# Julia-Tempering/Pigeons.jl

Measured on AMD Instinct MI355X. Metric: replica-steps/sec (explore+swap), toy_mvn d=1024, n_chains=1024; round-trip rate, higher is better.
Workload: dtype f64

## Files before the change

### pigeons.jl_amd/csrc/pte_slice8.hpp

```cpp
#pragma once
#include "pte_slice7.hpp"

namespace pte {

#ifndef PTE_S8_BD
#define PTE_S8_BD 3
#endif
#ifndef PTE_S8_BS
#define PTE_S8_BS 9
#endif
constexpr int S8_BD = PTE_S8_BD;

#ifndef PTE_S8_WAVES
#define PTE_S8_WAVES 4
#endif
template <int NLU, int S8_BS, int WINDOW, int DBL_MODE>
__device__ __forceinline__ void slice8_body(EngineDev e, SliceParams sp, const int64_t cl) {
    using namespace s7;
    constexpr int WIN = WINDOW, REFILL_AT = WINDOW - PTE_S7_MARGIN;
    constexpr bool FAST = (DBL_MODE == 2);
    static_assert(CAP_ITERS >= S8_BS, "lane 0 must be able to run past the speculative budget");
#ifndef PTE_S8_BLK
#define PTE_S8_BLK 256
#endif
    constexpr int BLK = PTE_S8_BLK, CPB = BLK / 64;
    constexpr bool HOLD_POLICY = (WIN == 512);
    __shared__ struct {
        double u[WIN];
        double e[WIN];
        double x[BLK];
        double we[256];
        unsigned long long ke[256];
        unsigned policy[HOLD_POLICY ? 2 : 0];
    } sm;
    double (&s_u)[WIN] = sm.u; double (&s_e)[WIN] = sm.e; double (&s_x)[BLK] = sm.x; double (&s_we)[256] = sm.we; unsigned long long (&s_ke)[256] = sm.ke;
    const int lane = lane_id();
#ifdef PTE_PROFILE_WAVES
    const uint64_t wave_t0 = __builtin_amdgcn_s_memrealtime();
#endif
    for (int i = lane; i < 256; i += 64) { s_we[i] = ZIG_WE[i]; s_ke[i] = ZIG_KE[i]; }
    if constexpr (HOLD_POLICY) sm.policy[0] = g_rng_policy;
    const auto exp_seq = [&](SeqRng &rs) __attribute__((always_inline)) -> double {
        if constexpr (HOLD_POLICY)
            return randexp_from_raw_hot(rs, rs.next(), [&]() __attribute__((always_inline)) -> unsigned {
                return (unsigned)__builtin_amdgcn_readfirstlane((int)*(const volatile __attribute__((address_space(3))) unsigned *)&sm.policy[0]); });
        else
            return randexp_seq(rs);
    };
    __syncthreads();
    if (cl >= e.K) return;
    const int64_t c = e.c0 + cl;
    const int slot = e.slot_of_chain[cl];
    if (is_ref_chain(e, c)) {
        iid_refresh_recorded<NLU>(e, cl, c, slot, e.sd[c], lane);
        return;
    }
    const double lp_before = lp_before_explore(e, c, slot);
    const int64_t d = e.d;
    double *xrow = e.x + (int64_t)slot * e.ld;
    const int B = (int)((d + 63) >> 6);
    const double nhp = e.nhp[c];
    const double inv_nhp = 1.0 / nhp;
    const double inv_abs_nhp = -inv_nhp * (1.0 + 1e-6);
    const double w = sp.w;
    const double w11 = 1.1 * sp.w;
    const int cap_iters = min(sp.max_iter, CAP_ITERS);
    const int kcap = min(sp.p, 20);
    const bool shr_more = S8_BS < cap_iters;
    constexpr bool HAND_SHRINK = (S8_BS == PTE_S8_BS && S8_BS >= 6 && S8_BS <= 10);
    constexpr bool N_IS_KN = (DBL_MODE == 2) && HAND_SHRINK;

    const int hg = s7_level(lane);
    const int hrel = s7_pick(LO, hg, 0) + lane - s7_pick(BASE, hg, 0);

    const int succ_lo = s7_pick(LO, hg + 1, 0), succ_wd = s7_pick(WD, hg + 1, 0), succ_base = s7_pick(BASE, hg + 1, 0);
    const int succ_off = hrel - succ_lo;
    const int word_c = 0x10000 - succ_off;
    const int word_c9 = (1 << 20) - succ_off * 512;
    const uint64_t seed_in = e.rng[2 * slot];

    double BS = 0.0;
    for (int b = 0; b < B; ++b) {
        int64_t i = 64 * (int64_t)b + lane;
        double v = (i < d) ? xrow[i] : 0.0;
        double s = wave_sum_dpp(v * v);
        if (lane == b) BS = s;
    }
    double S = upper_tree_root<NLU>(BS);
    if (nhp * S == -INFINITY) { if (lane == 0) set_error(e, ERR_SLICE_SUPPORT, (int)c, -1); return; }

    uint64_t wseed = e.rng[2 * slot];
    const uint64_t gamma = e.rng[2 * slot + 1];
    int p = 0;
    uint64_t gamma_inv = gamma;
    for (int k = 0; k < 5; ++k) gamma_inv *= 2ull - gamma * gamma_inv;
    double wsum = 0.0;
    typedef unsigned mask2_t __attribute__((ext_vector_type(2)));
    typedef unsigned slow_mask_t __attribute__((ext_vector_type(WIN / 32)));
    typedef double draws8_t __attribute__((ext_vector_type(8)));
    typedef double draws2_t __attribute__((ext_vector_type(2)));
    slow_mask_t slow_w;
    auto fill_window = [&]() __attribute__((always_inline)) {
        __syncthreads();
        double acc = 0.0;
#pragma unroll
        for (int k = 0; k < WIN / 64; ++k) {
            const int i = 64 * k + lane;
            const uint64_t r = mix64(wseed + (uint64_t)(i + 1) * gamma);
            const uint64_t ri = r & MASK52;
            const int idx = (int)(ri & 0xFF);
            const bool fast = ri < s_ke[idx];
            const double ev = (double)ri * s_we[idx];
            s_u[i] = u52_to_unit(r);
            s_e[i] = fast ? ev : __longlong_as_double(0x7ff8000000000000LL);
            acc += fast ? ev : 0.0;
            const uint64_t sb = ballot64(!fast);
            slow_w[2 * k] = (unsigned)sb; slow_w[2 * k + 1] = (unsigned)(sb >> 32);
        }
        wsum = wave_sum_dpp(acc);
        p = 0;
        __syncthreads();
    };
    fill_window();

    int dbl_z0 = 0, dbl_z1 = 0, dbl_one_hi = 0x3ff00000;
    if constexpr (DBL_MODE == 2) asm volatile("" : "+v"(dbl_z0), "+v"(dbl_z1), "+v"(dbl_one_hi));

    long long steps_sum = 0, fb_draws = 0, ex_total = 0;
    int steps_n = 0, acc_sum = 0, acc_n = 0, n_fb = 0;
    int err = 0, err_coord = -1;
#ifdef PTE_PROFILE_SECTIONS
    long long prof[20] = {0, 0, 0, 0, 0, 0, 0, 0, 0, 0, 0, 0, 0, 0, 0, 0, 0, 0, 0, 0};
#endif

    for (int pass = 0; pass < sp.n_passes && !err; ++pass) {
        for (int b = 0; BLK * (int64_t)b < d && !err; ++b) {
            const int64_t base = BLK * (int64_t)b;
            const int nl = (int)min((int64_t)BLK, d - base);
#pragma unroll
            for (int k = 0; k < CPB; ++k) s_x[64 * k + lane] = (64 * k + lane < nl) ? xrow[base + 64 * k + lane] : 0.0;
            __builtin_amdgcn_wave_barrier();
            double Sest = S * (1.0 + 1e-6) + wsum * inv_abs_nhp;
            int l = 0, l_end = nl;
            do {
                PROF_T(t0);
                if (__builtin_expect(p > REFILL_AT, 0)) { PROF_T(tr0); wseed += (uint64_t)p * gamma; fill_window(); Sest = Sest * (1.0 + 1e-6) + wsum * inv_abs_nhp; PROF_T(tr1); PROF_ADD(16, tr1 - tr0); PROF_ADD(17, 1); }
                const bool active = (l + hg) < nl;
                const double xold = s_x[(l + hg) & (BLK - 1)];
                int idx0 = p + hrel;
                double E = s_e[idx0];
                double u0 = s_u[idx0 + 1];
                double Vd[S8_BD];
#pragma unroll
                for (int it = 0; it < S8_BD; ++it) Vd[it] = s_u[idx0 + 2 + it];
                int ua = 0;
                if constexpr (DBL_MODE == 2) ua = (int)(uintptr_t)(const __attribute__((address_space(3))) double *)&s_u[idx0];
                int ex0 = 0;
                int cnt_base = 2;
                asm volatile("" : "+v"(cnt_base));
                if constexpr (DBL_MODE == 2) asm volatile("" : "+s"(ex0));
                unsigned slow_b;
                if constexpr (WIN == 512)
                    asm("s_lshr_b32 m0, %[p], 5\n" "s_nop 0\n" "s_movrels_b32 %[o], s84\n" "s_lshr_b32 %[o], %[o], %[p]"
                        : [o] "=&s"(slow_b) : [p] "s"(p), "{s[84:99]}"(slow_w) : "m0", "scc");
                else
                    asm("s_lshr_b32 m0, %[p], 5\n" "s_nop 0\n" "s_movrels_b32 %[o], s84\n" "s_lshr_b32 %[o], %[o], %[p]"
                        : [o] "=&s"(slow_b) : [p] "s"(p), "{s[84:91]}"(slow_w) : "m0", "scc");
                static_assert(WIN == 512 || WIN == 256, "the slow-path mask is sixteen or eight dwords");
                if (__builtin_expect((slow_b & 1u) != 0u, 0)) {
                    PROF_T(ts0);
                    SeqRng rs{wseed + (uint64_t)p * gamma, gamma};
                    const double Ex = exp_seq(rs);
                    const int used = (int)((rs.seed - (wseed + (uint64_t)p * gamma)) * gamma_inv);
                    if (used <= 17) {
                        ex0 = used - 1;
                        if (lane == 0) { E = Ex; idx0 += ex0; cnt_base = 2 + ex0; ua += 8 * ex0; }
                        Sest += Ex * inv_abs_nhp;
                        ex_total += ex0;
                        u0 = s_u[idx0 + 1];
#pragma unroll
                        for (int it = 0; it < S8_BD; ++it) Vd[it] = s_u[idx0 + 2 + it];
                    }
#ifdef PTE_PROFILE_SECTIONS
                    asm volatile("" :: "v"(E), "v"(u0), "v"(Vd[S8_BD - 1]), "v"(Sest));
#endif
                    PROF_T(ts1); PROF_ADD(18, ts1 - ts0); PROF_ADD(19, 1);
                }
                const double Enh = E * inv_nhp;
                const double Q = __builtin_fma(xold, xold, -Enh);
                const double Bq = Sest + fabs(Q);
                double dmin = fabs(Enh);
                auto test = [&](double v) __attribute__((always_inline)) -> double {
                    const double d = __builtin_fma(v, v, -Q);
                    dmin = fmin(dmin, fabs(d));
                    return d;
                };
                double LL = xold - w * u0;
                double RR = LL + w;
                double dL = test(LL), dR = test(RR);
                int kd = 0;
                double dmin_lr = 0.0;
                unsigned need_l0 = 0u;
                uint64_t need_m = 0ull;
                double thr2 = 0.0, mthr = 0.0, W = 0.0;
                int n = 0;
                uint64_t act_m = 0ull;
                draws8_t ud8 = 0.0; draws2_t ud2 = 0.0;
#if PTE_S8_BD >= 1 && PTE_S8_BD <= 4 && !defined(PTE_S8_DOUBLING_SELECTS)
                if constexpr (DBL_MODE == 2) {
                    double t_, wd_;
                    int sLh_, sRh_;
                    uint64_t sv_, sx_;
                    mask2_t sd_;
#define PTE_S8_CSTEP(V) \
                    "v_cmp_ge_f64 vcc, 0.5, " V "\n" \
                    "v_min_f64 v[102:103], v[114:115], v[116:117]\n" \
                    "v_cmpx_gt_f64_e64 %[sx], 0, v[102:103]\n" \
                    "v_add_f64 v[112:113], v[98:99], -v[96:97]\n" \
                    "v_add_u32 %[kd], 1, %[kd]\n" \
                    "v_add_u32 %[ua], 8, %[ua]\n" \
                    "v_cndmask_b32 v119, 0, %[one], vcc\n" \
                    "v_cndmask_b32 v121, %[one], v118, vcc\n" \
                    "v_fma_f64 v[96:97], -v[118:119], v[112:113], v[96:97]\n" \
                    "v_fma_f64 v[98:99], v[120:121], v[112:113], v[98:99]\n" \
                    "v_fma_f64 v[114:115], v[96:97], v[96:97], -v[110:111]\n" \
                    "v_fma_f64 v[116:117], v[98:99], v[98:99], -v[110:111]\n"
#define PTE_S8_CFOLD \
                    "v_min_f64 v[104:105], v[104:105], |v[114:115]|\n" \
                    "v_min_f64 v[104:105], v[104:105], |v[116:117]|\n"
#if PTE_S8_BS == 6
#define PTE_S8_UREADS_TAIL
#elif PTE_S8_BS == 7
#define PTE_S8_UREADS_TAIL "ds_read_b64 v[136:137], %[ua] offset:64\n"
#elif PTE_S8_BS == 8
#define PTE_S8_UREADS_TAIL "ds_read2_b64 v[136:139], %[ua] offset0:8 offset1:9\n"
#elif PTE_S8_BS == 9
#define PTE_S8_UREADS_TAIL "ds_read2_b64 v[136:139], %[ua] offset0:8 offset1:9\n" "ds_read_b64 v[140:141], %[ua] offset:80\n"
#else
#define PTE_S8_UREADS_TAIL "ds_read2_b64 v[136:139], %[ua] offset0:8 offset1:9\n" "ds_read2_b64 v[140:143], %[ua] offset0:10 offset1:11\n"
#endif
                    asm volatile("s_mov_b64 %[sv], exec\n"
#if PTE_S8_BD >= 2
                                 PTE_S8_CSTEP("%[V0]") PTE_S8_CFOLD
#endif
#if PTE_S8_BD >= 3
                                 PTE_S8_CSTEP("%[V1]") PTE_S8_CFOLD
#endif
#if PTE_S8_BD >= 4
                                 PTE_S8_CSTEP("%[V2]") PTE_S8_CFOLD
#endif
                                 PTE_S8_CSTEP("%[VL]")
                                 "s_mov_b64 exec, %[sv]\n"
                                 "ds_read2_b64 v[124:127], %[ua] offset0:2 offset1:3\n"
                                 "ds_read2_b64 v[128:131], %[ua] offset0:4 offset1:5\n"
                                 "ds_read2_b64 v[132:135], %[ua] offset0:6 offset1:7\n"
                                 PTE_S8_UREADS_TAIL
                                 "v_min_f64 v[102:103], v[114:115], v[116:117]\n"
                                 "v_cmp_gt_f64_e64 %[sd], 0, v[102:103]\n"
                                 PTE_S8_CFOLD
                                 "v_add_f64 %[mthr], %[Sest], |v[110:111]|\n"
                                 "v_max_f64 %[thr], |v[96:97]|, |v[98:99]|\n"
                                 "v_cmp_gt_i32_e64 %[act], %[nl], %[lg]\n"
                                 "v_add3_u32 v106, %[cb], %[so], %[kd]\n"
                                 "v_mul_f64 %[mthr], %[mthr], %[c_m]\n"
                                 "v_mul_f64 %[thr], %[thr], %[c_t]\n"
                                 "v_add_f64 v[112:113], v[98:99], -v[96:97]\n"
                                 : "+{v[96:97]}"(LL), "+{v[98:99]}"(RR), "+{v[114:115]}"(dL), "+{v[116:117]}"(dR), "+{v[104:105]}"(dmin), [kd] "+v"(kd), [ua] "+v"(ua),
                                   "=&{v[102:103]}"(t_), "=&{v[112:113]}"(wd_), "=&{v119}"(sLh_), "=&{v121}"(sRh_), [sv] "=&s"(sv_), [sx] "=&s"(sx_), [sd] "=&s"(sd_),
                                   "=&{v[124:139]}"(ud8), "=&{v[140:143]}"(ud2), [mthr] "=&v"(mthr), [thr] "=&v"(thr2), "=&{v106}"(n), [act] "=&s"(act_m)
                                 : "{v[110:111]}"(Q), "{v118}"(dbl_z0), "{v120}"(dbl_z1), [one] "v"(dbl_one_hi),
                                   [V0] "v"(Vd[0]), [V1] "v"(Vd[S8_BD > 2 ? 1 : 0]), [V2] "v"(Vd[S8_BD > 3 ? 2 : 0]), [VL] "v"(Vd[S8_BD - 1]),
                                   [Sest] "v"(Sest), [nl] "s"(nl), [lg] "v"(l + hg), [cb] "v"(cnt_base), [so] "v"(succ_off), [c_m] "s"(2e-12), [c_t] "s"(1e-6)
                                 : "vcc", "scc");
#undef PTE_S8_CSTEP
#undef PTE_S8_CFOLD
#undef PTE_S8_UREADS_TAIL
                    dmin_lr = t_; W = wd_;
                    need_m = (uint64_t)sd_.x | ((uint64_t)sd_.y << 32); need_l0 = __builtin_amdgcn_readfirstlane(sd_.x);
                } else
                if (DBL_MODE == 1 && sp.p >= S8_BD) {
                    double t_, wd_;
                    uint64_t sv_, sv2_;
#define PTE_S8_DSTEP(V) \
                    "v_min_f64 %[t], %[dL], %[dR]\n" \
                    "v_cmp_gt_f64 vcc, 0, %[t]\n" \
                    "s_and_saveexec_b64 %[sv], vcc\n" \
                    "v_add_u32 %[kd], 1, %[kd]\n" \
                    "v_add_f64 %[wd], %[RR], -%[LL]\n" \
                    "v_cmp_ge_f64 vcc, 0.5, " V "\n" \
                    "s_and_saveexec_b64 %[sv2], vcc\n" \
                    "v_add_f64 %[LL], %[LL], -%[wd]\n" \
                    "v_fma_f64 %[dL], %[LL], %[LL], -%[Q]\n" \
                    "v_min_f64 %[dmin], %[dmin], |%[dL]|\n" \
                    "s_andn2_b64 exec, %[sv2], exec\n" \
                    "v_add_f64 %[RR], %[RR], %[wd]\n" \
                    "v_fma_f64 %[dR], %[RR], %[RR], -%[Q]\n" \
                    "v_min_f64 %[dmin], %[dmin], |%[dR]|\n" \
                    "s_mov_b64 exec, %[sv]\n"
                    asm volatile(PTE_S8_DSTEP("%[V0]")
#if PTE_S8_BD >= 2
                                 PTE_S8_DSTEP("%[V1]")
#endif
#if PTE_S8_BD >= 3
                                 PTE_S8_DSTEP("%[V2]")
#endif
#if PTE_S8_BD >= 4
                                 PTE_S8_DSTEP("%[V3]")
#endif
                                 : [LL] "+v"(LL), [RR] "+v"(RR), [dL] "+v"(dL), [dR] "+v"(dR), [dmin] "+v"(dmin), [kd] "+v"(kd),
                                   [t] "=&v"(t_), [wd] "=&v"(wd_), [sv] "=&s"(sv_), [sv2] "=&s"(sv2_)
                                 : [Q] "v"(Q), [V0] "v"(Vd[0]), [V1] "v"(Vd[S8_BD > 1 ? 1 : 0]), [V2] "v"(Vd[S8_BD > 2 ? 2 : 0]), [V3] "v"(Vd[S8_BD > 3 ? 3 : 0])
                                 : "vcc", "scc");
#undef PTE_S8_DSTEP
                } else
#endif
#pragma unroll
                for (int it = 0; it < S8_BD; ++it) {
                    const bool need = (fmin(dL, dR) < 0.0) && it < sp.p;
                    const double V = Vd[it];
                    kd += need ? 1 : 0;
                    const bool left = V <= 0.5;
                    const double wd = RR - LL;
                    if constexpr (DBL_MODE == 0) {
                        const double sL = (need && left) ? 1.0 : 0.0, sR = (need && !left) ? 1.0 : 0.0;
                        LL = __builtin_fma(-sL, wd, LL);
                        RR = __builtin_fma(sR, wd, RR);
                        dL = __builtin_fma(LL, LL, -Q);
                        dR = __builtin_fma(RR, RR, -Q);
                        dmin = fmin(dmin, fmin(fabs(dL), fabs(dR)));
                    } else {
                        const double cand = left ? (LL - wd) : (RR + wd);
                        const double dc = __builtin_fma(cand, cand, -Q);
                        dmin = need ? fmin(dmin, fabs(dc)) : dmin;
                        const bool nl_ = need && left, nr_ = need && !left;
                        LL = nl_ ? cand : LL;
                        RR = nr_ ? cand : RR;
                        dL = nl_ ? dc : dL;
                        dR = nr_ ? dc : dR;
                    }
                }
#if !(PTE_S8_BD >= 1 && PTE_S8_BD <= 4) || defined(PTE_S8_DOUBLING_SELECTS)
                static_assert(DBL_MODE != 2, "PTE_S8_DBL_MODE == 2 needs the v_cmpx doubling block: 1 <= PTE_S8_BD <= 4 and no PTE_S8_DOUBLING_SELECTS");
#endif
                if constexpr (DBL_MODE != 2) dmin_lr = fmin(dL, dR);
                unsigned more_dbl;
                if constexpr (FAST) more_dbl = need_l0 & 1u;
                else more_dbl = ballot64(lane == 0 && (dmin_lr < 0.0) && kd < kcap) != 0ull ? 1u : 0u;
                if (__builtin_expect(more_dbl != 0u, 0)) {
                    bool need = (lane == 0);
                    while (need) {
                        const double V = s_u[idx0 + 2 + kd];
                        kd += 1;
                        const bool left = V <= 0.5;
                        const double wd = RR - LL;
                        const double cand = left ? (LL - wd) : (RR + wd);
                        const double dc = test(cand);
                        LL = left ? cand : LL;
                        RR = left ? RR : cand;
                        dL = left ? dc : dL;
                        dR = left ? dR : dc;
                        need = (kd < kcap) && (fmin(dL, dR) < 0.0);
                    }
                    asm volatile("" : "+v"(dL), "+v"(dR), "+v"(kd));
                    dmin_lr = fmin(dL, dR);
                    if constexpr (FAST) {
                        dmin_lr = (kd >= sp.p) ? 0.0 : dmin_lr;
                        need_m = ballot64(dmin_lr < 0.0);
                        need_l0 = (unsigned)need_m;
                        thr2 = 1e-6 * fmax(fabs(LL), fabs(RR));
                        n = cnt_base + kd + succ_off;
                        W = RR - LL;
                        const double *un = &s_u[idx0 + 2 + kd];
#pragma unroll
                        for (int k = 0; k < 8; ++k) ud8[k] = (k < S8_BS) ? un[k] : 0.0;
#pragma unroll
                        for (int k = 8; k < 10; ++k) ud2[k - 8] = (k < S8_BS) ? un[k] : 0.0;
                        asm volatile("" : "+{v[124:139]}"(ud8), "+{v[140:143]}"(ud2));
                    }
                }
                const bool dbl_ok = FAST ? !__builtin_amdgcn_inverse_ballot_w64(need_m) : !((kd < sp.p) && (dmin_lr < 0.0));
                if constexpr (DBL_MODE != 2) thr2 = 1e-6 * fmax(fabs(LL), fabs(RR));
#ifdef PTE_PROFILE_SECTIONS
                asm volatile("" :: "v"(LL), "v"(RR), "v"(kd), "v"(thr2));
#endif
                PROF_T(t1); PROF_ADD(0, t1 - t0);
                static_assert(DBL_MODE != 2 || HAND_SHRINK, "PTE_S8_DBL_MODE == 2 hands its draws to the hand-written shrinkage block: 6 <= PTE_S8_BS <= 10");
                const double *us = &s_u[idx0 + 2 + kd];
                double u[S8_BS];
                if constexpr (DBL_MODE != 2) {
#pragma unroll
                    for (int k = 0; k < S8_BS; ++k) u[k] = us[k];
                }
                if constexpr (DBL_MODE != 2) mthr = 2e-12 * Bq;
                int kn0 = cnt_base + kd + succ_off;
                uint64_t pre_ok;
                if constexpr (FAST) pre_ok = 0ull;
                else pre_ok = ballot64(active && dbl_ok);
                double Lbar = LL, Rbar = RR, xf = xold;
                if constexpr (!N_IS_KN) n = 0;
                bool fin = false;
                unsigned unf_l0 = 0u;
                uint64_t unf_m = 0ull;
                if constexpr (S8_BS == PTE_S8_BS && S8_BS >= 6 && S8_BS <= 10) {
                    double t_;
                    mask2_t unf_mask;
                    uint64_t exec_save;
#define PTE_S8_STEP_W \
                    "v_add_f64 v[112:113], v[98:99], -v[96:97]\n"
#define PTE_S8_STEP(U) PTE_S8_STEP_W PTE_S8_STEP_U(U)
#define PTE_S8_STEP_U(U) \
                    "v_mul_f64 v[102:103], " U ", v[112:113]\n" \
                    "v_add_f64 v[100:101], v[96:97], v[102:103]\n" \
                    "v_cmp_lt_f64 vcc, v[100:101], v[108:109]\n" \
                    "v_fma_f64 v[102:103], v[100:101], v[100:101], -v[110:111]\n" \
                    "v_add_u32 v106, 1, v106\n" \
                    "v_cndmask_b32 v96, v96, v100, vcc\n" \
                    "v_cndmask_b32 v97, v97, v101, vcc\n" \
                    "v_cndmask_b32 v98, v100, v98, vcc\n" \
                    "v_cndmask_b32 v99, v101, v99, vcc\n" \
                    "v_min_f64 v[104:105], v[104:105], |v[102:103]|\n" \
                    "v_cmpx_ngt_f64 vcc, 0, v[102:103]\n"
                    if constexpr (DBL_MODE == 2) {
#if defined(PTE_S8_ONE_WAIT) || defined(PTE_PROFILE_SECTIONS)
#define PTE_S8_WAIT(K) "s_waitcnt lgkmcnt(0)\n"
#else
#define PTE_S8_WAIT(K) "s_waitcnt lgkmcnt(" #K ")\n"
#endif
#if PTE_S8_BS >= 9
#define PTE_S8_W1 4
#define PTE_S8_W3 3
#define PTE_S8_W5 2
#define PTE_S8_W7 1
#elif PTE_S8_BS >= 7
#define PTE_S8_W1 3
#define PTE_S8_W3 2
#define PTE_S8_W5 1
#define PTE_S8_W7 0
#else
#define PTE_S8_W1 2
#define PTE_S8_W3 1
#define PTE_S8_W5 0
#endif
#define PTE_S8_WAIT_(K) PTE_S8_WAIT(K)
                    asm volatile(".p2align 3\n"
                                 "s_mov_b64 %[sv], exec\n"
                                 "s_andn2_b64 %[pre], %[act], %[need]\n"
                                 PTE_S8_WAIT_(PTE_S8_W1) PTE_S8_STEP_U("v[124:125]") PTE_S8_STEP("v[126:127]")
                                 PTE_S8_STEP_W PTE_S8_WAIT_(PTE_S8_W3) PTE_S8_STEP_U("v[128:129]") PTE_S8_STEP("v[130:131]")
                                 PTE_S8_STEP_W PTE_S8_WAIT_(PTE_S8_W5) PTE_S8_STEP_U("v[132:133]") PTE_S8_STEP("v[134:135]")
#if PTE_S8_BS >= 7
                                 PTE_S8_STEP_W PTE_S8_WAIT_(PTE_S8_W7) PTE_S8_STEP_U("v[136:137]")
#endif
#if PTE_S8_BS >= 8
                                 PTE_S8_STEP("v[138:139]")
#endif
#if PTE_S8_BS >= 9
                                 PTE_S8_STEP_W PTE_S8_WAIT_(0) PTE_S8_STEP_U("v[140:141]")
#endif
#if PTE_S8_BS >= 10
                                 PTE_S8_STEP("v[142:143]")
#endif
                                 "s_mov_b64 %[unf], exec\n"
                                 "s_mov_b64 exec, %[sv]\n"
                                 "s_nop 3\n"
                                 : "+{v[96:97]}"(Lbar), "+{v[98:99]}"(Rbar), "=&{v[100:101]}"(xf), "=&{v[102:103]}"(t_),
                                   "+{v[104:105]}"(dmin), "+{v106}"(n), "+{v[112:113]}"(W), [unf] "=&s"(unf_mask), [sv] "=&s"(exec_save), [pre] "=&s"(pre_ok)
                                 : "{v[108:109]}"(xold), "{v[110:111]}"(Q), "{v[124:139]}"(ud8), "{v[140:143]}"(ud2), [act] "s"(act_m), [need] "s"(need_m)
                                 : "vcc", "scc");
#undef PTE_S8_WAIT
#undef PTE_S8_WAIT_
#undef PTE_S8_W1
#undef PTE_S8_W3
#undef PTE_S8_W5
#undef PTE_S8_W7
                    } else
                    asm volatile(".p2align 3\n"
                                 "s_mov_b64 %[sv], exec\n"
                                 PTE_S8_STEP("%[u0]") PTE_S8_STEP("%[u1]") PTE_S8_STEP("%[u2]") PTE_S8_STEP("%[u3]")
                                 PTE_S8_STEP("%[u4]") PTE_S8_STEP("%[u5]")
#if PTE_S8_BS >= 7
                                 PTE_S8_STEP("%[u6]")
#endif
#if PTE_S8_BS >= 8
                                 PTE_S8_STEP("%[u7]")
#endif
#if PTE_S8_BS >= 9
                                 PTE_S8_STEP("%[u8]")
#endif
#if PTE_S8_BS >= 10
                                 PTE_S8_STEP("%[u9]")
#endif
                                 "s_mov_b64 %[unf], exec\n"
                                 "s_mov_b64 exec, %[sv]\n"
                                 "s_nop 3\n"
                                 : "+{v[96:97]}"(Lbar), "+{v[98:99]}"(Rbar), "=&{v[100:101]}"(xf), "=&{v[102:103]}"(t_),
                                   "+{v[104:105]}"(dmin), "+{v106}"(n), "=&{v[112:113]}"(W), [unf] "=&s"(unf_mask), [sv] "=&s"(exec_save)
                                 : "{v[108:109]}"(xold), "{v[110:111]}"(Q), [u0] "v"(u[0]), [u1] "v"(u[1]), [u2] "v"(u[2]), [u3] "v"(u[3]),
                                   [u4] "v"(u[4]), [u5] "v"(u[5]), [u6] "v"(u[S8_BS > 6 ? 6 : 0]), [u7] "v"(u[S8_BS > 7 ? 7 : 0]),
                                   [u8] "v"(u[S8_BS > 8 ? 8 : 0]), [u9] "v"(u[S8_BS > 9 ? 9 : 0])
                                 : "vcc");
#undef PTE_S8_STEP
#undef PTE_S8_STEP_W
#undef PTE_S8_STEP_U
                    unf_m = (uint64_t)unf_mask.x | ((uint64_t)unf_mask.y << 32); unf_l0 = __builtin_amdgcn_readfirstlane(unf_mask.x);
                    fin = !__builtin_amdgcn_inverse_ballot_w64(unf_m);
                } else {
#pragma unroll
                    for (int k = 0; k < S8_BS; ++k) {
                        W = Rbar - Lbar;
                        const double v = Lbar + u[k] * W;
                        const double dv = __builtin_fma(v, v, -Q);
                        dmin = fmin(dmin, fabs(dv));
                        xf = fin ? xf : v;
                        n += fin ? 0 : 1;
                        const bool below = v < xold;
                        Lbar = below ? v : Lbar;
                        Rbar = below ? Rbar : v;
                        fin = fin || (dv < 0.0);
                    }
                    unf_m = ballot64(!fin);
                    unf_l0 = (unsigned)unf_m;
                }
                if (__builtin_expect((unf_l0 & 1u) != 0u, 0)) {
                  if (shr_more) {
                    double dx = 1.0;
                    bool go = (lane == 0);
                    const int n_off = N_IS_KN ? cnt_base + kd + succ_off : 0;
                    while (go) {
                        W = Rbar - Lbar;
                        xf = Lbar + us[n - n_off] * W;
                        n += 1;
                        dx = test(xf);
                        const bool below = xf < xold;
                        Lbar = below ? xf : Lbar;
                        Rbar = below ? Rbar : xf;
                        go = !(dx < 0.0) && n - n_off < cap_iters;
                    }
                    asm volatile("" : "+v"(dx), "+v"(n), "+v"(W));
                    fin = fin || (lane == 0 && dx < 0.0);
                    unf_m = ballot64(!fin);
                  }
                }
                PROF_T(t2); PROF_ADD(1, t2 - t1); PROF_ADD(3, 1);
                int gdone;
#ifdef PTE_PROFILE_SECTIONS
                constexpr bool ASM_TAIL = false;
#else
                constexpr bool ASM_TAIL = FAST && G == 5;
#endif
                if constexpr (ASM_TAIL) {
                    const int kn = N_IS_KN ? n : kn0 + n;
                    const int wsucc = ((unsigned)kn < (unsigned)succ_wd) ? kn + succ_base : 0;
                    const int word_v = (kn << 9) + word_c9 + wsucc;
                    unsigned acc; uint64_t tmask, sA_, sB_; int w_, pk_, s0_, s1_, s2_, s3_, s4_;
                    asm volatile("v_cmp_gt_f64 vcc, %[W], %[thr]\n"
                                 "v_cndmask_b32_e64 %[w], 0, %[wv], %[pre]\n"
                                 "v_cmp_gt_f64_e64 %[sA], %[dm], %[mthr]\n"
                                 "v_cndmask_b32_e64 %[w], %[w], 0, %[unf]\n"
                                 "v_cndmask_b32_e32 %[w], 0, %[w], vcc\n"
                                 "s_nop 0\n"
                                 "v_cndmask_b32_e64 %[w], 0, %[w], %[sA]\n"
                                 "v_cndmask_b32_e64 %[pk], 0, %[w], %[nz]\n"
                                 : [w] "=&v"(w_), [pk] "=&v"(pk_), [sA] "=&s"(sA_)
                                 : [wv] "v"(word_v), [pre] "s"(pre_ok), [unf] "s"(unf_m), [nz] "s"(0xFFFFFFFFFFFFFFFEull),
                                   [W] "v"(W), [thr] "v"(thr2), [dm] "v"(dmin), [mthr] "v"(mthr)
                                 : "vcc");
                    asm volatile("v_cmp_ne_u32_e64 %[sB], 0, %[w]\n"
                                 "s_mov_b64 %[tm], 1\n"
                                 "v_readlane_b32 %[s0], %[w], 0\n"
                                 "s_nop 3\n"
                                 "v_readlane_b32 %[s1], %[pk], %[s0]\n"
                                 "s_bitset1_b64 %[tm], %[s0]\n"
                                 "s_mov_b32 %[acc], %[s0]\n"
                                 "s_nop 1\n"
                                 "v_readlane_b32 %[s2], %[pk], %[s1]\n"
                                 "s_bitset1_b64 %[tm], %[s1]\n"
                                 "s_add_u32 %[acc], %[acc], %[s1]\n"
                                 "s_nop 1\n"
                                 "v_readlane_b32 %[s3], %[pk], %[s2]\n"
                                 "s_bitset1_b64 %[tm], %[s2]\n"
                                 "s_add_u32 %[acc], %[acc], %[s2]\n"
                                 "s_nop 1\n"
                                 "v_readlane_b32 %[s4], %[pk], %[s3]\n"
                                 "s_bitset1_b64 %[tm], %[s3]\n"
                                 "s_add_u32 %[acc], %[acc], %[s3]\n"
                                 "s_and_b64 %[tm], %[tm], %[sB]\n"
                                 "s_add_u32 %[acc], %[acc], %[s4]\n"
                                 : [sB] "=&s"(sB_), [tm] "=&s"(tmask), [acc] "=&s"(acc),
                                   [s0] "=&s"(s0_), [s1] "=&s"(s1_), [s2] "=&s"(s2_), [s3] "=&s"(s3_), [s4] "=&s"(s4_)
                                 : [w] "v"(w_), [pk] "v"(pk_)
                                 : "scc");
                    if (__builtin_amdgcn_inverse_ballot_w64(tmask)) s_x[(l + hg) & (BLK - 1)] = xf;
                    __builtin_amdgcn_wave_barrier();
                    p += (int)((acc >> 9) & 0x1FFu);
                    gdone = (int)((acc >> 20) & 7u);
                    l += gdone;
                } else {
                bool valid = __builtin_amdgcn_inverse_ballot_w64(pre_ok) && fin && (W > thr2);
                if constexpr (!FAST) valid = valid && !(E != E) && n <= cap_iters;
#ifdef PTE_PROFILE_SECTIONS
                asm volatile("" :: "v"(xf), "v"(n), "v"(dmin));
#endif
#ifdef PTE_PROFILE_SECTIONS
                {
                    const bool mg = dmin > 2e-12 * Bq;
                    const int rc = !active ? 7 : (E != E) ? 1 : !dbl_ok ? 2 : !fin ? 3 : !valid ? 4 : !mg ? 5 : 0;
                    const int cnt_ = N_IS_KN ? n - succ_off : cnt_base + kd + n;
                    int o_ = 0, g_ = 0, why = 0;
                    for (g_ = 0; g_ < G; ++g_) {
                        if (l + g_ >= nl) { why = 7; break; }
                        const int k_ = o_ - LO[g_];
                        if ((unsigned)k_ >= (unsigned)WD[g_]) { why = 6; break; }
                        const int ln_ = BASE[g_] + k_;
                        const int r_ = __builtin_amdgcn_readlane(rc, ln_);
                        if (r_) { why = r_; break; }
                        o_ += __builtin_amdgcn_readlane(cnt_, ln_);
                    }
                    PROF_ADD(8 + why, 1);
                }
#endif
                valid = valid && (dmin > mthr);
                const int kn = N_IS_KN ? n : kn0 + n;
                const bool inw = (unsigned)kn < (unsigned)succ_wd;
                const uint64_t vmask = ballot64(valid);
                int word_v = kn + word_c + (inw ? (int)((unsigned)(kn + succ_base) << 24) : 0);
                asm("" : "+v"(word_v));
                const int word = valid ? word_v : 0;
                const int packed = (lane != 0) ? word : 0;
#ifdef PTE_PROFILE_SECTIONS
                asm volatile("" :: "v"(packed));
#endif
                {
                    int pk = __builtin_amdgcn_readlane(word, 0);
                    unsigned acc = 0u;
                    uint64_t tmask = 1ull;
#pragma unroll
                    for (int g = 1; g < G; ++g) {
                        const int cur = (int)((unsigned)pk >> 24);
                        asm volatile("s_bitset1_b64 %0, %2\n\ts_add_u32 %1, %1, %3" : "+s"(tmask), "+s"(acc) : "s"(cur), "s"(pk) : "scc");
                        pk = __builtin_amdgcn_readlane(packed, cur);
                    }
                    acc += (unsigned)pk;
                    tmask &= vmask;
                    if (__builtin_amdgcn_inverse_ballot_w64(tmask)) s_x[(l + hg) & (BLK - 1)] = xf;
                    __builtin_amdgcn_wave_barrier();
                    p += (int)(acc & 0xFFFFu);
                    gdone = (int)((acc >> 16) & 0xFFu);
                    l += gdone;
                }
                }
#ifdef PTE_PROFILE_SECTIONS
                asm volatile("" :: "s"(p), "s"(l));
#endif
                PROF_T(t4); PROF_ADD(5, t4 - t2); PROF_ADD(4, gdone);
                if (__builtin_expect(gdone == 0, 0)) {
                    ex_total -= ex0;
                    SeqRng rs{wseed + (uint64_t)p * gamma, gamma};
                    const int ck = l >> 6, li = l & 63, bc = CPB * b + ck;
#pragma unroll
                    for (int k = 0; k < CPB; ++k) {
                        const double xk = s_x[64 * k + lane];
                        const double sk = wave_sum_dpp(xk * xk);
                        if (lane == CPB * b + k) BS = sk;
                    }
                    const double X = s_x[64 * ck + lane];
                    const double xo = readlane_f64(X, li);
                    const double E = exp_seq(rs);
                    const double u0 = rs.rand();
                    const double Q = xo * xo - E * inv_nhp;
                    const double mg = 1e-12 * (Sest + fabs(Q));
                    const double Qlo = Q - mg, Qhi = Q + mg;
                    auto inside_exact = [&](double v) __attribute__((always_inline)) -> bool {
                        const double Xv = (lane == li) ? v : X;
                        const double sv = wave_sum_dpp(Xv * Xv), s0 = wave_sum_dpp(X * X);
                        const double Sv = upper_tree_root<NLU>((lane == bc) ? sv : BS);
                        const double S0 = upper_tree_root<NLU>((lane == bc) ? s0 : BS);
                        const double zz = nhp * S0 - E;
                        return zz < nhp * Sv;
                    };
                    auto inside = [&](double v) __attribute__((always_inline)) -> bool {
                        const double q = v * v;
                        const bool in = q < Qlo;
                        const bool out = q > Qhi;
                        if (__builtin_expect(!(in || out), 0)) return inside_exact(v);
                        return in;
                    };
                    double LL = xo - w * u0;
                    double RR = LL + w;
                    bool in_L = inside(LL), in_R = inside(RR);
                    int K = sp.p;
                    while (K > 0 && (in_L || in_R)) {
                        const double V = rs.rand();
                        if (V <= 0.5) { LL = LL - (RR - LL); in_L = inside(LL); }
                        else { RR = RR + (RR - LL); in_R = inside(RR); }
                        K -= 1;
                    }
                    steps_sum += (sp.p - K); steps_n += 1;
                    const bool doubled = (RR - LL) > w11;
                    double Lbar = LL, Rbar = RR;
                    double xn = xo;
                    bool fin = false;
                    for (int n = 1; n <= sp.max_iter; ++n) {
                        const double newpos = Lbar + rs.rand() * (Rbar - Lbar);
                        if (inside(newpos)) {
                            bool ok = true;
                            if (doubled) {
                                double Lhat = LL, Rhat = RR;
                                bool oL = !in_L, oR = !in_R;
                                bool Rstale = false, Lstale = false, D = false;
                                while (Rhat - Lhat > w11) {
                                    const double Mid = (Lhat + Rhat) / 2.0;
                                    if ((xo < Mid && newpos >= Mid) || (xo >= Mid && newpos < Mid)) D = true;
                                    if (newpos < Mid) { Rhat = Mid; Rstale = true; }
                                    else { Lhat = Mid; Lstale = true; }
                                    if (D) {
                                        if (Lstale) { oL = !inside(Lhat); Lstale = false; }
                                        if (Rstale) { oR = !inside(Rhat); Rstale = false; }
                                        if (oL && oR) { ok = false; break; }
                                    }
                                }
                            }
                            acc_n += 1;
                            if (ok) { acc_sum += 1; xn = newpos; steps_sum += n; steps_n += 1; fin = true; break; }
                        }
                        if (newpos < xo) Lbar = newpos; else Rbar = newpos;
                        if (jl_isapprox(Lbar, Rbar)) { steps_sum += n; steps_n += 1; fin = true; break; }
                    }
                    if (!fin) { err = ERR_SLICE_MAX_ITER; err_coord = (int)(base + l); l_end = 0; continue; }
                    Sest = Sest + fabs(xn * xn - xo * xo);
                    if (lane == li) s_x[l] = xn;
                    __builtin_amdgcn_wave_barrier();
                    l += 1;
                    const int used = (int)((rs.seed - (wseed + (uint64_t)p * gamma)) * gamma_inv);
                    p += used;
                    fb_draws += used; n_fb += 1;
                    PROF_T(t5); PROF_ADD(7, t5 - t4); PROF_ADD(6, 1);
                }
            } while (l < l_end);
            if (err) break;
            {
#pragma unroll
                for (int k = 0; k < CPB; ++k) {
                    const double X = s_x[64 * k + lane];
                    if (64 * k + lane < nl) xrow[base + 64 * k + lane] = X;
                    const double s = wave_sum_dpp(X * X);
                    if (lane == CPB * b + k) BS = s;
                }
                S = upper_tree_root<NLU>(BS);
                if (__builtin_expect(!isfinite(nhp * S), 0)) { err = ERR_SLICE_INVALID_LP; err_coord = (int)base; }
            }
        }
    }
    if (err) { if (lane == 0) set_error(e, err, (int)c, err_coord); return; }
    if (lane == 0) {
        const uint64_t seed_out = wseed + (uint64_t)p * gamma;
        const long long n_spec = (long long)sp.n_passes * d - n_fb;
        const long long spec_draws = (long long)((seed_out - seed_in) * gamma_inv) - fb_draws;
        steps_sum += spec_draws - ex_total - 2 * n_spec; steps_n += (int)(2 * n_spec); acc_sum += (int)n_spec; acc_n += (int)n_spec;
        e.suff[slot] = S;
        e.rng[2 * slot] = seed_out;
        e.expl_steps_sum[cl] += (double)steps_sum; e.expl_steps_n[cl] += steps_n;
        e.expl_acc_sum[cl] += (double)acc_sum;     e.expl_acc_n[cl] += acc_n;
#ifdef PTE_PROFILE_SECTIONS
        for (int i = 0; i < 20; ++i) e.on_m2[20 * cl + i] += (double)prof[i];
#endif
    }
    record_after_explore(e, cl, c, slot, lane, lp_before, S, 0.0);
#ifdef PTE_PROFILE_WAVES
    if (lane == 0) {
        double *o = e.on_m2 + 2 * (e.d + 1) + 4 * cl;
        o[0] = (double)wave_t0; o[1] = (double)__builtin_amdgcn_s_memrealtime();
        o[2] = (double)__builtin_amdgcn_s_getreg((31 << 11) | 4); o[3] = (double)__builtin_amdgcn_s_getreg((31 << 11) | 20);
    }
#endif
}

#ifndef PTE_S8_DBL_MODE
#define PTE_S8_DBL_MODE 2
#endif
template <int NLU, int S8_BS>
__global__ __launch_bounds__(64) __attribute__((amdgpu_waves_per_eu(PTE_S8_WAVES, PTE_S8_WAVES))) void k_explore_slice8(EngineDev e, SliceParams sp) {
    slice8_body<NLU, S8_BS, PTE_S7_WIN, PTE_S8_DBL_MODE>(e, sp, blockIdx.x);
}
template <int NLU, int S8_BS>
__global__ __launch_bounds__(64) __attribute__((amdgpu_waves_per_eu(PTE_S8_WAVES, PTE_S8_WAVES))) void k_explore_slice8_generic(EngineDev e, SliceParams sp) {
    slice8_body<NLU, S8_BS, PTE_S7_WIN, 0>(e, sp, blockIdx.x);
}
#ifndef PTE_S8_TWIN_WAVES
#define PTE_S8_TWIN_WAVES PTE_S8_WAVES
#endif
#ifndef PTE_S8_TWIN_FROM
#define PTE_S8_TWIN_FROM (256 * 8)
#endif
template <int NLU, int S8_BS>
__global__ __launch_bounds__(64) __attribute__((amdgpu_waves_per_eu(PTE_S8_TWIN_WAVES, PTE_S8_TWIN_WAVES))) void k_explore_slice8_lds10k(EngineDev e, SliceParams sp) {
    slice8_body<NLU, S8_BS, 256, 1>(e, sp, blockIdx.x);
}

template <int NLU, int S8_BS, int WINDOW, int DBL_MODE>
__device__ __forceinline__ void slice8_scan_loop(EngineDev e, const SliceParams &sp, const ScanLoop &sl) {
    const int lane = lane_id();
    const int64_t cl = scan_loop_chain(e.K);
    int go = 1;
    if (lane == 0) go = scan_loop_gate(sl) ? 1 : 0;
    if (!__builtin_amdgcn_readfirstlane(go)) return;
    for (int64_t i = 0; i < sl.n_scans; ++i) {
        e.trace_idx = sl.scan_idx0 + i;
        slice8_body<NLU, S8_BS, WINDOW, DBL_MODE>(e, sp, cl);
        __syncthreads();
        int slot = 0;
        if (lane == 0) slot = swap_handshake(e, sl, i, cl, e.slot_of_chain[cl]);
        slot = __builtin_amdgcn_readfirstlane(slot);
        __syncthreads();
        if (slot < 0) return;
    }
}
template <int NLU, int S8_BS>
__global__ __launch_bounds__(64) __attribute__((amdgpu_waves_per_eu(PTE_S8_WAVES, PTE_S8_WAVES))) void k_scans_slice8(EngineDev e, SliceParams sp, ScanLoop sl) {
    slice8_scan_loop<NLU, S8_BS, PTE_S7_WIN, PTE_S8_DBL_MODE>(e, sp, sl);
}
template <int NLU, int S8_BS>
__global__ __launch_bounds__(64) __attribute__((amdgpu_waves_per_eu(PTE_S8_WAVES, PTE_S8_WAVES))) void k_scans_slice8_generic(EngineDev e, SliceParams sp, ScanLoop sl) {
    slice8_scan_loop<NLU, S8_BS, PTE_S7_WIN, 0>(e, sp, sl);
}
}
```

Baseline: 1.693 million.

## Precompute ziggurat slow-path exponential draws during window fill for window 512

During window refill, each lane records the last slow-path ziggurat draw it owns. It resolves it in parallel, using either the wedge test or the next-draw tail, and caches the result and the draw count in shared memory. In the serial slice loop, a slow-path hit at position p reads the cached resolution when it matches and skips the sequential exp_seq fallback. This adds an exp() and some LDS traffic per refill, plus an extra barrier, in exchange for fewer serial sequential-RNG fallbacks. It only applies when the window is 512 (HOLD_POLICY).

```diff
diff --git a/pigeons.jl_amd/csrc/pte_slice8.hpp b/pigeons.jl_amd/csrc/pte_slice8.hpp
--- a/pigeons.jl_amd/csrc/pte_slice8.hpp
+++ b/pigeons.jl_amd/csrc/pte_slice8.hpp
@@ -32,6 +32,8 @@
         double we[256];
         unsigned long long ke[256];
         unsigned policy[HOLD_POLICY ? 2 : 0];
+        double rex[HOLD_POLICY ? 64 : 0];
+        unsigned rmeta[HOLD_POLICY ? 64 : 0];
     } sm;
     double (&s_u)[WIN] = sm.u; double (&s_e)[WIN] = sm.e; double (&s_x)[BLK] = sm.x; double (&s_we)[256] = sm.we; unsigned long long (&s_ke)[256] = sm.ke;
     const int lane = lane_id();
@@ -100,9 +102,15 @@
     typedef double draws8_t __attribute__((ext_vector_type(8)));
     typedef double draws2_t __attribute__((ext_vector_type(2)));
     slow_mask_t slow_w;
+#ifdef PTE_PROFILE_SECTIONS
+    long long prof[21] = {0, 0, 0, 0, 0, 0, 0, 0, 0, 0, 0, 0, 0, 0, 0, 0, 0, 0, 0, 0, 0};
+#endif
+    constexpr unsigned S8_UNRESOLVED = 0xFFFFu;
     auto fill_window = [&]() __attribute__((always_inline)) {
         __syncthreads();
         double acc = 0.0;
+        double pend_x = 0.0;
+        int pend_m = WIN;
 #pragma unroll
         for (int k = 0; k < WIN / 64; ++k) {
             const int i = 64 * k + lane;
@@ -116,10 +124,27 @@
             acc += fast ? ev : 0.0;
             const uint64_t sb = ballot64(!fast);
             slow_w[2 * k] = (unsigned)sb; slow_w[2 * k + 1] = (unsigned)(sb >> 32);
+            if constexpr (HOLD_POLICY) { pend_x = fast ? pend_x : ev; pend_m = fast ? pend_m : (i | (idx << 16)); }
         }
         wsum = wave_sum_dpp(acc);
         p = 0;
         __syncthreads();
+        if constexpr (HOLD_POLICY) {
+            __builtin_amdgcn_sched_barrier(0);
+            const int pi = pend_m & 0xFFFF, pidx = pend_m >> 16;
+            const double f1 = ZIG_FE[pidx], f0 = ZIG_FE[(pidx - 1) & 0xFF];
+            const double un = s_u[min(pi + 1, WIN - 1)], en = s_e[min(pi + 2, WIN - 1)];
+            const double ex = exp(-pend_x);
+            const bool in_reach = (pidx != 0) && (pi + 2 < WIN);
+            const bool wedge = (f0 - f1) * un + f1 < ex;
+            const unsigned used = !in_reach ? 0u : wedge ? 2u : (en == en) ? 3u : 0u;
+            sm.rex[lane] = wedge ? pend_x : en;
+            sm.rmeta[lane] = used ? ((unsigned)pi | (used << 16)) : S8_UNRESOLVED;
+#ifdef PTE_PROFILE_SECTIONS
+            prof[20] += (long long)__popcll(ballot64(used != 0u)) << 24;
+#endif
+            __syncthreads();
+        }
     };
     fill_window();
 
@@ -129,9 +154,6 @@
     long long steps_sum = 0, fb_draws = 0, ex_total = 0;
     int steps_n = 0, acc_sum = 0, acc_n = 0, n_fb = 0;
     int err = 0, err_coord = -1;
-#ifdef PTE_PROFILE_SECTIONS
-    long long prof[20] = {0, 0, 0, 0, 0, 0, 0, 0, 0, 0, 0, 0, 0, 0, 0, 0, 0, 0, 0, 0};
-#endif
 
     for (int pass = 0; pass < sp.n_passes && !err; ++pass) {
         for (int b = 0; BLK * (int64_t)b < d && !err; ++b) {
@@ -169,6 +191,35 @@
                 static_assert(WIN == 512 || WIN == 256, "the slow-path mask is sixteen or eight dwords");
                 if (__builtin_expect((slow_b & 1u) != 0u, 0)) {
                     PROF_T(ts0);
+                    if constexpr (HOLD_POLICY) {
+                        const auto head_moves = [&](const double Ex, const int used) __attribute__((always_inline)) {
+                            ex0 = used - 1;
+                            if (lane == 0) { E = Ex; idx0 += ex0; cnt_base = 2 + ex0; ua += 8 * ex0; }
+                            Sest += Ex * inv_abs_nhp;
+                            ex_total += ex0;
+                            u0 = s_u[idx0 + 1];
+#pragma unroll
+                            for (int it = 0; it < S8_BD; ++it) Vd[it] = s_u[idx0 + 2 + it];
+                        };
+                        const unsigned rmeta = (unsigned)__builtin_amdgcn_readfirstlane((int)sm.rmeta[p & 63]);
+                        const double rex = sm.rex[p & 63];
+                        if ((rmeta & 0xFFFFu) == (unsigned)p) {
+                            head_moves(rex, (int)(rmeta >> 16));
+#ifdef PTE_PROFILE_SECTIONS
+                            asm volatile("" :: "v"(E), "v"(u0), "v"(Vd[S8_BD - 1]), "v"(Sest));
+#endif
+                            PROF_T(ts1); PROF_ADD(2, ts1 - ts0); PROF_ADD(20, 1);
+                        } else {
+                            SeqRng rs{wseed + (uint64_t)p * gamma, gamma};
+                            const double Ex = exp_seq(rs);
+                            const int used = (int)((rs.seed - (wseed + (uint64_t)p * gamma)) * gamma_inv);
+                            if (used <= 17) head_moves(Ex, used);
+#ifdef PTE_PROFILE_SECTIONS
+                            asm volatile("" :: "v"(E), "v"(u0), "v"(Vd[S8_BD - 1]), "v"(Sest));
+#endif
+                            PROF_T(ts1); PROF_ADD(18, ts1 - ts0); PROF_ADD(19, 1);
+                        }
+                    } else {
                     SeqRng rs{wseed + (uint64_t)p * gamma, gamma};
                     const double Ex = exp_seq(rs);
                     const int used = (int)((rs.seed - (wseed + (uint64_t)p * gamma)) * gamma_inv);
@@ -185,6 +236,7 @@
                     asm volatile("" :: "v"(E), "v"(u0), "v"(Vd[S8_BD - 1]), "v"(Sest));
 #endif
                     PROF_T(ts1); PROF_ADD(18, ts1 - ts0); PROF_ADD(19, 1);
+                    }
                 }
                 const double Enh = E * inv_nhp;
                 const double Q = __builtin_fma(xold, xold, -Enh);
@@ -762,7 +814,7 @@
         e.expl_steps_sum[cl] += (double)steps_sum; e.expl_steps_n[cl] += steps_n;
         e.expl_acc_sum[cl] += (double)acc_sum;     e.expl_acc_n[cl] += acc_n;
 #ifdef PTE_PROFILE_SECTIONS
-        for (int i = 0; i < 20; ++i) e.on_m2[20 * cl + i] += (double)prof[i];
+        for (int i = 0; i < 21; ++i) e.on_m2[21 * cl + i] += (double)prof[i];
 #endif
     }
     record_after_explore(e, cl, c, slot, lane, lp_before, S, 0.0);
```

After: 1.753 million, median of 6. 1.04x the previous value.
